# Sunscreen-tech/spf

Measured on AMD Instinct MI355X. Metric: programmable bootstraps/sec (CMUX gates/sec) at default 128-bit params, higher is better.
Workload: dtype f64

## Files before the change

spf_amd/csrc/spf_device.hpp:

```cpp
#pragma once
#include <hip/hip_runtime.h>
#include <stdint.h>

namespace spf {

struct c64 {
    double re, im;
};

typedef double f64x2_t __attribute__((ext_vector_type(2)));
typedef const f64x2_t __attribute__((address_space(1)))* gc64_ptr;
typedef const uint64_t __attribute__((address_space(1)))* gu64_cptr;
typedef uint64_t __attribute__((address_space(1)))* gu64_ptr;
__device__ __forceinline__ gc64_ptr global_view(const c64* p) { return (gc64_ptr)(uintptr_t)p; }
__device__ __forceinline__ gu64_cptr global_view(const uint64_t* p) { return (gu64_cptr)(uintptr_t)p; }
__device__ __forceinline__ gu64_ptr global_view(uint64_t* p) { return (gu64_ptr)(uintptr_t)p; }
__device__ __forceinline__ c64 gload(gc64_ptr p) { f64x2_t v = *p; return {v.x, v.y}; }
__device__ __forceinline__ c64 gload_stream(gc64_ptr p) { f64x2_t v = __builtin_nontemporal_load(p); return {v.x, v.y}; }

__device__ __forceinline__ c64 cadd(c64 a, c64 b) { return {a.re + b.re, a.im + b.im}; }
__device__ __forceinline__ c64 csub(c64 a, c64 b) { return {a.re - b.re, a.im - b.im}; }

__device__ __forceinline__ c64 cmul_nf(c64 a, c64 b)
{
    c64 o;
    o.re = a.re * b.re - a.im * b.im;
    o.im = a.re * b.im + a.im * b.re;
    return o;
}
__device__ __forceinline__ c64 cmul_nf_conj(c64 a, c64 b)
{
    c64 o;
    o.re = a.re * b.re + a.im * b.im;
    o.im = a.im * b.re - a.re * b.im;
    return o;
}

template <int DIR> __device__ __forceinline__ c64 cmul_tw(c64 a, c64 w)
{
    c64 o;
    if (DIR > 0) {
        double t1 = a.im * w.im;
        o.re = __builtin_fma(a.re, w.re, -t1);
        double t2 = a.im * w.re;
        o.im = __builtin_fma(a.re, w.im, t2);
    } else {
        double t1 = a.im * w.im;
        o.re = __builtin_fma(a.re, w.re, t1);
        double t2 = a.im * w.re;
        o.im = __builtin_fma(-a.re, w.im, t2);
    }
    return o;
}

constexpr double kSqrtHalf = 0.70710678118654752440;

template <int DIR> __device__ __forceinline__ void radix8(c64 (&v)[8])
{
    c64 s0 = cadd(v[0], v[4]), s1 = cadd(v[1], v[5]), s2 = cadd(v[2], v[6]), s3 = cadd(v[3], v[7]);
    c64 t0 = csub(v[0], v[4]), t1 = csub(v[1], v[5]), t2 = csub(v[2], v[6]), t3 = csub(v[3], v[7]);
    c64 t1w, t3w;
    if (DIR > 0) {
        double p1 = t1.re + t1.im, m1 = t1.im - t1.re;
        t1w.re = p1 * kSqrtHalf; t1w.im = m1 * kSqrtHalf;
        double p3 = t3.re + t3.im, m3 = t3.im - t3.re;
        t3w.re = m3 * kSqrtHalf; t3w.im = -(p3 * kSqrtHalf);
    } else {
        double p1 = t1.re + t1.im, m1 = t1.re - t1.im;
        t1w.re = m1 * kSqrtHalf; t1w.im = p1 * kSqrtHalf;
        double p3 = t3.re + t3.im, m3 = t3.re - t3.im;
        t3w.re = -(p3 * kSqrtHalf); t3w.im = m3 * kSqrtHalf;
    }
    c64 a0 = cadd(s0, s2), a1 = cadd(s1, s3), a2 = csub(s0, s2), d = csub(s1, s3);
    v[0] = cadd(a0, a1);
    v[4] = csub(a0, a1);
    c64 b0, b2;
    if (DIR > 0) {
        v[2] = {a2.re + d.im, a2.im - d.re};
        v[6] = {a2.re - d.im, a2.im + d.re};
        b0 = {t0.re + t2.im, t0.im - t2.re};
        b2 = {t0.re - t2.im, t0.im + t2.re};
    } else {
        v[2] = {a2.re - d.im, a2.im + d.re};
        v[6] = {a2.re + d.im, a2.im - d.re};
        b0 = {t0.re - t2.im, t0.im + t2.re};
        b2 = {t0.re + t2.im, t0.im - t2.re};
    }
    c64 b1 = cadd(t1w, t3w), e = csub(t1w, t3w);
    v[1] = cadd(b0, b1);
    v[5] = csub(b0, b1);
    if (DIR > 0) {
        v[3] = {b2.re + e.im, b2.im - e.re};
        v[7] = {b2.re - e.im, b2.im + e.re};
    } else {
        v[3] = {b2.re - e.im, b2.im + e.re};
        v[7] = {b2.re + e.im, b2.im - e.re};
    }
}

constexpr int kT1Off = 0;
constexpr int kT2Off = kT1Off + 7 * 64;
constexpr int kWCOff = kT2Off + 7 * 8;
constexpr int kTWOff = kWCOff + 512;
constexpr int kTableEntries = kTWOff + 1024;
constexpr int kTableBytes = kTableEntries * 16;
constexpr int kWaveBufBytes = 16384;

__device__ __forceinline__ void wave_lds_fence()
{
    asm volatile("s_waitcnt lgkmcnt(0)" ::: "memory");
}
__device__ __forceinline__ void compiler_fence() { asm volatile("" ::: "memory"); }
__device__ __forceinline__ void sched_fence()
{
    asm volatile("" ::: "memory");
    __builtin_amdgcn_sched_barrier(0);
}

template <int DIR, int PRE = 0>
__device__ __forceinline__ void fft512_single(c64 (&V)[8], char* buf, const c64* tab, int lane)
{
    const int hi3 = lane >> 3, lo3 = lane & 7;
    const int rd = 16 * (8 * lo3 + (hi3 ^ lo3));
    {
        c64 tw[PRE > 0 ? PRE : 1];
#pragma unroll
        for (int k = 0; k < PRE; k++) tw[k] = tab[kT1Off + k * 64 + lane];
        if constexpr (PRE > 0) compiler_fence();
        radix8<DIR>(V);
#pragma unroll
        for (int k1 = 1; k1 < 8; k1++)
            V[k1] = cmul_tw<DIR>(V[k1], (k1 - 1 < PRE) ? tw[k1 - 1 < PRE ? k1 - 1 : 0] : tab[kT1Off + (k1 - 1) * 64 + lane]);
    }
#pragma unroll
    for (int k1 = 0; k1 < 8; k1++)
        *reinterpret_cast<c64*>(buf + 16 * (64 * hi3 + 8 * k1 + (lo3 ^ k1))) = V[k1];
    wave_lds_fence();
    {
        c64 tw[PRE > 0 ? PRE : 1];
#pragma unroll
        for (int k = 0; k < PRE; k++) tw[k] = tab[kT2Off + k * 8 + hi3];
#pragma unroll
        for (int a = 0; a < 8; a++) V[a] = *reinterpret_cast<const c64*>(buf + 1024 * a + rd);
        if constexpr (PRE > 0) compiler_fence();
        radix8<DIR>(V);
#pragma unroll
        for (int c = 1; c < 8; c++)
            V[c] = cmul_tw<DIR>(V[c], (c - 1 < PRE) ? tw[c - 1 < PRE ? c - 1 : 0] : tab[kT2Off + (c - 1) * 8 + hi3]);
    }
    compiler_fence();
#pragma unroll
    for (int c = 0; c < 8; c++)
        *reinterpret_cast<c64*>(buf + 16 * (64 * hi3 + 8 * lo3 + (c ^ lo3))) = V[c];
    wave_lds_fence();
#pragma unroll
    for (int b = 0; b < 8; b++) V[b] = *reinterpret_cast<const c64*>(buf + 1024 * b + rd);
    radix8<DIR>(V);
    compiler_fence();
}

__device__ __forceinline__ void swap_halves32(double& a, double& b)
{
    uint32_t al = (uint32_t)__double2loint(a), ah = (uint32_t)__double2hiint(a);
    uint32_t bl = (uint32_t)__double2loint(b), bh = (uint32_t)__double2hiint(b);
    auto r0 = __builtin_amdgcn_permlane32_swap(al, bl, false, false);
    auto r1 = __builtin_amdgcn_permlane32_swap(ah, bh, false, false);
    a = __hiloint2double((int)r1[0], (int)r0[0]);
    b = __hiloint2double((int)r1[1], (int)r0[1]);
}
__device__ __forceinline__ void swap_rows16(double& a, double& b)
{
    uint32_t al = (uint32_t)__double2loint(a), ah = (uint32_t)__double2hiint(a);
    uint32_t bl = (uint32_t)__double2loint(b), bh = (uint32_t)__double2hiint(b);
    auto r0 = __builtin_amdgcn_permlane16_swap(al, bl, false, false);
    auto r1 = __builtin_amdgcn_permlane16_swap(ah, bh, false, false);
    a = __hiloint2double((int)r1[0], (int)r0[0]);
    b = __hiloint2double((int)r1[1], (int)r0[1]);
}
__device__ __forceinline__ void swap_lane8(double& a, double& b)
{
    constexpr int kRowRor8 = 0x128;
    int al = __double2loint(a), ah = __double2hiint(a);
    int bl = __double2loint(b), bh = __double2hiint(b);
    int nal = __builtin_amdgcn_update_dpp(al, bl, kRowRor8, 0xF, 0xC, false);
    int nah = __builtin_amdgcn_update_dpp(ah, bh, kRowRor8, 0xF, 0xC, false);
    int nbl = __builtin_amdgcn_update_dpp(bl, al, kRowRor8, 0xF, 0x3, false);
    int nbh = __builtin_amdgcn_update_dpp(bh, ah, kRowRor8, 0xF, 0x3, false);
    a = __hiloint2double(nah, nal);
    b = __hiloint2double(nbh, nbl);
}
__device__ __forceinline__ void lane_transpose_hi3(c64 (&V)[8])
{
#pragma unroll
    for (int r = 0; r < 4; r++) {
        swap_halves32(V[r].re, V[r + 4].re);
        swap_halves32(V[r].im, V[r + 4].im);
    }
#pragma unroll
    for (int r = 0; r < 8; r++) {
        if (r & 2) continue;
        swap_rows16(V[r].re, V[r + 2].re);
        swap_rows16(V[r].im, V[r + 2].im);
    }
#pragma unroll
    for (int r = 0; r < 8; r += 2) {
        swap_lane8(V[r].re, V[r + 1].re);
        swap_lane8(V[r].im, V[r + 1].im);
    }
}

template <int DIR>
__device__ __forceinline__ void fft512_pair_pipelined(c64 (&E)[8], c64 (&O)[8], char* bufE, char* bufO,
                                                      const c64* tab, int lane)
{
    const int hi3 = lane >> 3, lo3 = lane & 7;
    const int rd = 16 * (8 * lo3 + (hi3 ^ lo3));
    c64 tw1[7], tw2[7];
#pragma unroll
    for (int k1 = 1; k1 < 8; k1++) tw1[k1 - 1] = tab[kT1Off + (k1 - 1) * 64 + lane];
#pragma unroll
    for (int c = 1; c < 8; c++) tw2[c - 1] = tab[kT2Off + (c - 1) * 8 + hi3];
    compiler_fence();
    radix8<DIR>(E);
#pragma unroll
    for (int k1 = 1; k1 < 8; k1++) E[k1] = cmul_tw<DIR>(E[k1], tw1[k1 - 1]);
#pragma unroll
    for (int k1 = 0; k1 < 8; k1++)
        *reinterpret_cast<c64*>(bufE + 16 * (64 * hi3 + 8 * k1 + (lo3 ^ k1))) = E[k1];
    compiler_fence();
#pragma unroll
    for (int a = 0; a < 8; a++) E[a] = *reinterpret_cast<const c64*>(bufE + 1024 * a + rd);
    compiler_fence();
    radix8<DIR>(O);
#pragma unroll
    for (int k1 = 1; k1 < 8; k1++) O[k1] = cmul_tw<DIR>(O[k1], tw1[k1 - 1]);
#pragma unroll
    for (int k1 = 0; k1 < 8; k1++)
        *reinterpret_cast<c64*>(bufO + 16 * (64 * hi3 + 8 * k1 + (lo3 ^ k1))) = O[k1];
    compiler_fence();
#pragma unroll
    for (int a = 0; a < 8; a++) O[a] = *reinterpret_cast<const c64*>(bufO + 1024 * a + rd);
    compiler_fence();
    radix8<DIR>(E);
#pragma unroll
    for (int c = 1; c < 8; c++) E[c] = cmul_tw<DIR>(E[c], tw2[c - 1]);
#pragma unroll
    for (int c = 0; c < 8; c++)
        *reinterpret_cast<c64*>(bufE + 16 * (64 * hi3 + 8 * lo3 + (c ^ lo3))) = E[c];
    compiler_fence();
#pragma unroll
    for (int b = 0; b < 8; b++) E[b] = *reinterpret_cast<const c64*>(bufE + 1024 * b + rd);
    compiler_fence();
    radix8<DIR>(O);
#pragma unroll
    for (int c = 1; c < 8; c++) O[c] = cmul_tw<DIR>(O[c], tw2[c - 1]);
#pragma unroll
    for (int c = 0; c < 8; c++)
        *reinterpret_cast<c64*>(bufO + 16 * (64 * hi3 + 8 * lo3 + (c ^ lo3))) = O[c];
    compiler_fence();
#pragma unroll
    for (int b = 0; b < 8; b++) O[b] = *reinterpret_cast<const c64*>(bufO + 1024 * b + rd);
    compiler_fence();
    radix8<DIR>(E);
    radix8<DIR>(O);
    compiler_fence();
// ... 266 lines not shown
#pragma unroll
    for (int k = 0; k < 7; k++) tw[k] = tab[kT1Off + k * 64 + lane];
    compiler_fence();
    radix8<DIR>(A);
#pragma unroll
    for (int k1 = 1; k1 < 8; k1++) A[k1] = cmul_tw<DIR>(A[k1], tw[k1 - 1]);
    sched_fence();
    radix8_twr_spread<DIR>(B, tw, [&](int k) { store(A, k); });
    load(A, rd1);
    sched_fence();
#pragma unroll
    for (int c = 0; c < 7; c++) tw[c] = tab[kT2Off + c * 8 + hi3];
    compiler_fence();
    radix8_twr_spread<DIR>(A, tw, [&](int k) { store(B, k); });
    mid();
    load(B, rd1);
    sched_fence();
    radix8_twr_spread<DIR>(B, tw, [&](int k) { store(A, k); });
    load(A, rd2);
    sched_fence();
    if constexpr (XP == 2) {
        lane_transpose_hi3(B);
        radix8<DIR>(A);
        radix8<DIR>(B);
    } else {
        pair_tail_through_image<DIR>(A, B, store, load, rd2);
    }
    sched_fence();
}
template <int DIR, int XP = 2, class MID = no_hook>
__device__ __forceinline__ void fft512_pair1ts2(c64 (&A)[8], c64 (&B)[8], char* buf, const c64* tab, int lane, MID mid = MID())
{
    static_assert(XP == 2 || XP == 0, "exchange 2 of B in registers (2) or through the image behind A's (0)");
    const int hi3 = lane >> 3, lo3 = lane & 7;
    const uint32_t rd1 = 16 * (8 * lo3 + (hi3 ^ lo3));
    const uint32_t rd2 = 16 * (8 * hi3 + (hi3 ^ lo3));
    const uint32_t wbase = 16 * (64 * hi3 + lo3);
    char* wr[8];
#pragma unroll
    for (int r = 0; r < 8; r++) wr[r] = buf + ((wbase ^ (16 * r)) + 128 * r);
    auto store = [&](c64 (&X)[8], int k) { *reinterpret_cast<c64*>(wr[k]) = X[k]; };
    auto load = [&](c64 (&X)[8], uint32_t rd) {
#pragma unroll
        for (int a = 0; a < 8; a++) X[a] = *reinterpret_cast<const c64*>(buf + 1024 * a + rd);
    };
    c64 tw[7];
#pragma unroll
    for (int k = 0; k < 7; k++) tw[k] = tab[kT1Off + k * 64 + lane];
    compiler_fence();
    radix8<DIR>(A);
#pragma unroll
    for (int k1 = 1; k1 < 8; k1++) A[k1] = cmul_tw<DIR>(A[k1], tw[k1 - 1]);
    sched_fence();
    radix8_twr_spread2<DIR>(B, tw, [&](int k) { store(A, k); }, [&]() { load(A, rd1); });
    c64 tw2[7];
#pragma unroll
    for (int c = 0; c < 7; c++) tw2[c] = tab[kT2Off + c * 8 + hi3];
    compiler_fence();
    radix8_twr_spread2<DIR>(A, tw2, [&](int k) { store(B, k); }, [&]() { load(B, rd1); });
    mid();
    radix8_twr_spread2<DIR>(B, tw2, [&](int k) { store(A, k); }, [&]() { load(A, rd2); });
    if constexpr (XP == 2) {
        lane_transpose_hi3(B);
        radix8<DIR>(A);
        radix8<DIR>(B);
    } else {
        pair_tail_through_image<DIR>(A, B, store, load, rd2);
    }
    sched_fence();
}

__device__ __forceinline__ uint64_t f64_round_to_torus(double x)
{
    const double q = 18446744073709551616.0;
    const double q_div_2 = 9223372036854775808.0;
    double v = __builtin_round(x);
    double m = __builtin_fma(-__builtin_trunc(v * (1.0 / q)), q, v);
    double adj = (m >= q_div_2) ? -q : ((m <= -q_div_2) ? q : 0.0);
    m += adj;
    bool sat = m >= q_div_2;
    long long r = (long long)(sat ? 0.0 : m);
    r = sat ? 0x7FFFFFFFFFFFFFFFll : r;
    return (uint64_t)r;
}

__device__ __forceinline__ uint64_t f64_bigint_to_torus_bits(double v, uint32_t& sh_or, uint32_t& quirk_min)
{
    const uint64_t b = (uint64_t)__double_as_longlong(v);
    const uint32_t hi = (uint32_t)(b >> 32), lo = (uint32_t)b;
    const uint32_t sh = ((hi >> 20) & 0x7FFu) - 1075u;
    sh_or |= sh;
    const uint64_t m = ((uint64_t)((hi & 0xFFFFFu) | 0x100000u) << 32) | lo;
    uint64_t r = m << (sh & 63u);
    const uint32_t s32 = (uint32_t)((int32_t)hi >> 31);
    const uint64_t s = ((uint64_t)s32 << 32) | s32;
    r = (r ^ s) - s;
    const uint32_t q = (uint32_t)r | ((uint32_t)(r >> 32) ^ 0x80000000u) | ~s32;
    quirk_min = q < quirk_min ? q : quirk_min;
    return r;
}

__device__ __forceinline__ void torus_bits16_mantissa(const double (&tv)[16], uint64_t (&t)[16])
{
    uint32_t sh_or = 0, qmin = 0xFFFFFFFFu;
#pragma unroll
    for (int e = 0; e < 16; e++) t[e] = f64_bigint_to_torus_bits(tv[e], sh_or, qmin);
    if (!__all(sh_or < 64u && qmin != 0u)) {
#pragma unroll
        for (int e = 0; e < 16; e++) t[e] = f64_round_to_torus(tv[e]);
    }
}
__device__ __forceinline__ void torus_bits16(const double (&tv)[16], uint64_t (&t)[16])
{
    uint32_t emin = 0xFFFFFFFFu, emax = 0u;
    uint64_t quirk = 0;
#pragma unroll
    for (int e = 0; e < 16; e++) {
        const uint64_t b = (uint64_t)__double_as_longlong(tv[e]);
        const uint32_t hi = (uint32_t)(b >> 32);
        const uint32_t e11 = (hi >> 20) & 0x7FFu;
        emin = e11 < emin ? e11 : emin;
        emax = e11 > emax ? e11 : emax;
        const uint64_t r = b << ((e11 + 13u) & 63u);
        quirk |= __ballot((uint32_t)(r >> 32) == 0x80000000u);
        const uint32_t s32 = (uint32_t)((int32_t)hi >> 31);
        const uint64_t sg = ((uint64_t)s32 << 32) | s32;
        t[e] = (r ^ sg) - sg;
    }
    if (!__all(emin >= 1087u && emax <= 1138u) || quirk != 0) {
#pragma unroll
        for (int e = 0; e < 16; e++) t[e] = f64_round_to_torus(tv[e]);
    }
}
template <bool MANTISSA_FORM = false>
__device__ __forceinline__ void untwist_to_torus_bits(const c64 (&V)[8], const c64* twist_lds, uint64_t (&t)[16])
{
    double tv[16];
#pragma unroll
    for (int n1 = 0; n1 < 8; n1++) {
        c64 xs = {V[n1].re * (1.0 / 1024.0), V[n1].im * (1.0 / 1024.0)};
        c64 u = cmul_nf_conj(xs, twist_lds[64 * n1]);
        tv[n1] = u.re;
        tv[8 + n1] = u.im;
    }
    if constexpr (MANTISSA_FORM) torus_bits16_mantissa(tv, t);
    else torus_bits16(tv, t);
}
__device__ __forceinline__ uint64_t add_u32_to_u64(uint64_t a, uint32_t b)
{
    uint64_t out, carry;
    asm("v_mad_u64_u32 %0, %1, %2, 1, %3" : "=&v"(out), "=s"(carry) : "v"(b), "v"(a));
    return out;
}

template <bool TWIST_AT_ONCE = false>
__device__ __forceinline__ void untwist_sub_from_negated(const c64 (&V)[8], const c64* twist_lds, uint64_t (&nacc)[16])
{
    double tvn[16];
    c64 twf[TWIST_AT_ONCE ? 8 : 1];
    if constexpr (TWIST_AT_ONCE) {
#pragma unroll
        for (int n1 = 0; n1 < 8; n1++) twf[n1] = twist_lds[64 * n1];
        compiler_fence();
    }
#pragma unroll
    for (int n1 = 0; n1 < 8; n1++) {
        const c64 xs = V[n1];
        const c64 tw = TWIST_AT_ONCE ? twf[TWIST_AT_ONCE ? n1 : 0] : twist_lds[64 * n1];
        tvn[n1] = -(xs.re * tw.re) - xs.im * tw.im;
        tvn[8 + n1] = xs.re * tw.im - xs.im * tw.re;
    }
    uint32_t kmin = 0xFFFFFFFFu, kmax = 0u;
    int32_t qmin = 0x7FFFFFFF;
    uint64_t t[16];
#pragma unroll
    for (int e = 0; e < 16; e++) {
        const uint64_t b = (uint64_t)__double_as_longlong(tvn[e]);
        const uint32_t hi = (uint32_t)(b >> 32);
        const uint32_t k = hi << 1;
        kmin = k < kmin ? k : kmin;
        kmax = k > kmax ? k : kmax;
        const uint64_t r = b << (((hi >> 20) + 13u) & 63u);
        const int32_t rh = (int32_t)(uint32_t)(r >> 32);
        qmin = rh < qmin ? rh : qmin;
        const uint64_t sg = (uint64_t)((int64_t)b >> 63);
        t[e] = (r + sg) ^ sg;
    }
    if (__all(kmin >= (1087u << 21) && kmax < (1139u << 21) && qmin != (int32_t)0x80000000)) {
#pragma unroll
        for (int e = 0; e < 16; e++) nacc[e] += t[e];
    } else {
#pragma unroll
        for (int e = 0; e < 16; e++) nacc[e] -= f64_round_to_torus(-tvn[e]);
    }
}
__device__ __forceinline__ void untwist_to_torus_bits(const c64 (&V)[8], const c64 (&twist)[8], uint64_t (&t)[16])
{
    double tv[16];
#pragma unroll
    for (int n1 = 0; n1 < 8; n1++) {
        c64 xs = {V[n1].re * (1.0 / 1024.0), V[n1].im * (1.0 / 1024.0)};
        c64 u = cmul_nf_conj(xs, twist[n1]);
        tv[n1] = u.re;
        tv[8 + n1] = u.im;
    }
    torus_bits16(tv, t);
}


template <int L, int LOGB>
__device__ __forceinline__ uint32_t gadget_digits_packed(uint64_t x)
{
    static_assert(L * LOGB <= 32, "packed digits need L*LOGB <= 32");
    constexpr int shift = 64 - L * LOGB;
    uint32_t s = (uint32_t)(x >> shift) + (uint32_t)((x >> (shift - 1)) & 1);
    uint32_t packed = 0;
#pragma unroll
    for (int j = 0; j < L; j++) {
        uint32_t d = s & ((1u << LOGB) - 1);
        s >>= LOGB;
        s += d >> (LOGB - 1);
        packed |= d << (j * LOGB);
    }
    return packed;
}

__device__ __forceinline__ c64 twisted_digit_top32(uint32_t s_re, uint32_t s_im, int j, c64 tw)
{
    const int dre = j == 0 ? (int)(int16_t)(s_re & 0xFFFFu) : (int)(s_re + 0x8000u) >> 16;
    const int dim = j == 0 ? (int)(int16_t)(s_im & 0xFFFFu) : (int)(s_im + 0x8000u) >> 16;
    return cmul_nf({(double)dre, (double)dim}, tw);
}

template <int LOGB>
__device__ __forceinline__ c64 twisted_digit(uint32_t packed_re, uint32_t packed_im, int j, c64 tw)
{
    const int sh = j * LOGB;
    int dre = ((int)(packed_re << (32 - LOGB - sh))) >> (32 - LOGB);
    int dim = ((int)(packed_im << (32 - LOGB - sh))) >> (32 - LOGB);
    return cmul_nf({(double)dre, (double)dim}, tw);
}

}
```

spf_amd/csrc/spf_kernels.hpp:

```cpp
#pragma once
#include <type_traits>
#include "spf_device.hpp"

namespace spf {

constexpr int kN = 2048;
constexpr int kHalf = 1024;
constexpr int kWavesPerBlock = 4;

struct BlindRotateArgs {
    const uint64_t* lwe_in;
    const uint64_t* lut;
    size_t lut_stride;
    const c64* bsk;
    const c64* tables;
    uint64_t* out;
    size_t out_stride;
    uint32_t n;
    uint32_t B;
    uint32_t log_chi, log_v;
    uint64_t body_rotate;
    uint32_t sample_extract;
    uint64_t* stamps;
};

__device__ __forceinline__ uint32_t mod_switch_2n(uint64_t x, uint32_t log_chi, uint32_t log_v)
{
    const uint32_t log_modulus = 12;
    x = x << log_chi;
    uint32_t shift = 64 - (log_modulus - log_v);
    uint64_t round = (x >> (shift - 1)) & 1;
    x = x >> shift;
    return (uint32_t)(((x + round) & ((1u << log_modulus) - 1)) << log_v);
}

constexpr int kBskSlotBytes = 2 * kHalf * 16;

__device__ __forceinline__ void lds_dma_piece(const void* sbase, uint32_t voff, uint32_t lds)
{
    uint32_t saved_m0;
    asm volatile("s_mov_b32 %0, m0\n\ts_mov_b32 m0, %3\n\ts_nop 0\n\tglobal_load_lds_dwordx4 %1, %2\n\ts_mov_b32 m0, %0"
                 : "=&s"(saved_m0) : "v"(voff), "s"(sbase), "s"(lds) : "memory");
}
__device__ __forceinline__ uint32_t lds_address(const void* p)
{
    return (uint32_t)(size_t)(const __attribute__((address_space(3))) void*)p;
}

template <int NT>
__device__ __forceinline__ void table_image_dma(const c64* tables, char* smem, int tid, int wv)
{
    const char* src = reinterpret_cast<const char*>(tables);
    const uint32_t voff = (uint32_t)tid * 16u;
    const uint32_t dst = lds_address(smem) + (uint32_t)wv * 1024u;
    constexpr int kRow = NT * 16, kFull = kTableBytes / kRow, kRest = kTableBytes - kFull * kRow;
#pragma unroll
    for (int k = 0; k < kFull; k++) lds_dma_piece(src + k * kRow, voff, dst + k * kRow);
    if constexpr (kRest > 0) {
        if (tid * 16 < kRest) lds_dma_piece(src + kFull * kRow, voff, dst + kFull * kRow);
    }
}

__device__ __forceinline__ void pair_barrier_w()
{
    asm volatile("s_waitcnt lgkmcnt(0)" ::: "memory");
    __builtin_amdgcn_s_barrier();
    asm volatile("" ::: "memory");
}

constexpr int kBlindRotate2pLds = kTableBytes + 4 * kWaveBufBytes + 2 * kBskSlotBytes;

template <int PRIO>
__device__ __forceinline__ void young_prio(uint32_t flag) {
    uint32_t tmp;
    if constexpr (PRIO != 0)
        asm volatile("v_readfirstlane_b32 %0, %1\n\ts_cmp_eq_u32 %0, 0\n\ts_cbranch_scc1 .Lprio%=\n\ts_setprio 1\n.Lprio%=:" : "=&s"(tmp) : "v"(flag) : "scc");
    else
        asm volatile("v_readfirstlane_b32 %0, %1\n\ts_cmp_eq_u32 %0, 0\n\ts_cbranch_scc1 .Lprio%=\n\ts_setprio 0\n.Lprio%=:" : "=&s"(tmp) : "v"(flag) : "scc");
}

#ifndef SPF_PRIO_SCHED_EVEN
#define SPF_PRIO_SCHED_EVEN "----00----10--1-----"
#endif
#ifndef SPF_PRIO_SCHED_MIX
#define SPF_PRIO_SCHED_MIX "----1-----1---10-00-"
#endif
template <int MIX> constexpr char prio_sched_at(int i) { return MIX ? SPF_PRIO_SCHED_MIX[i] : SPF_PRIO_SCHED_EVEN[i]; }
static_assert(sizeof(SPF_PRIO_SCHED_EVEN) == 21 && sizeof(SPF_PRIO_SCHED_MIX) == 21, "20 schedule points");

#ifndef SPF_PAIR_E0
#define SPF_PAIR_E0 fft512_pair1ts2
#endif
#ifndef SPF_PAIR_E1
#define SPF_PAIR_E1 fft512_pair1ts
#endif
#ifndef SPF_PAIR_EI
#define SPF_PAIR_EI fft512_pair1ts2
#endif
#ifndef SPF_PAIR_M0
#define SPF_PAIR_M0 fft512_pair1ts
#endif
#ifndef SPF_PAIR_M1
#define SPF_PAIR_M1 fft512_pair1ts
#endif
#ifndef SPF_PAIR_MI
#define SPF_PAIR_MI fft512_pair1ts
#endif
#ifndef SPF_BR_OPT
#define SPF_BR_OPT 6
#endif
#ifndef SPF_BR_OPT_MIX
#define SPF_BR_OPT_MIX 10
#endif
#ifndef SPF_BR2_OPT
#define SPF_BR2_OPT 6
#endif
template <int L, int LOGB, int OPT, int W, int CTS = 4, int MIX = 1>
__device__ __forceinline__ void blind_rotate2p_body(const BlindRotateArgs& a, char* smem)
{
    constexpr int XP = (OPT & 1) ? 1 : ((OPT & 2) ? 2 : 0);
#ifdef SPF_STAMPS
    uint64_t st_acc[12] = {0, 0, 0, 0, 0, 0, 0, 0, 0, 0, 0, 0};
    uint64_t st_prev = __builtin_amdgcn_s_memtime();
#define STAMP(i) do { uint64_t t_ = __builtin_amdgcn_s_memtime(); st_acc[i] += t_ - st_prev; st_prev = t_; } while (0)
#else
#define STAMP(i) do { } while (0)
#endif
    static_assert(L == 2 && LOGB == 16, "two 16-bit digits, taken straight from the rounded top word and processed as a pair");
    constexpr int NT = 128 * CTS;
    c64* tab = reinterpret_cast<c64*>(smem);
    const int tid = threadIdx.x;
    const int lane = tid & 63;
    const int wv = __builtin_amdgcn_readfirstlane(tid >> 6);
    const int cslot = wv >> 1;
    constexpr int w = W;
    char* tile = smem + kTableBytes + cslot * kWaveBufBytes;
    char* mine = tile + w * 8192;
    char* theirs = tile + (w ^ 1) * 8192;
    char* bskring = smem + kTableBytes + CTS * kWaveBufBytes;

    {
        const double2* src = reinterpret_cast<const double2*>(a.tables);
        double2* dst = reinterpret_cast<double2*>(smem);
        for (int i = tid; i < kTableEntries; i += NT) dst[i] = src[i];
    }

    const uint32_t ct_raw = blockIdx.x * CTS + cslot;
    const bool owns_output = ct_raw < a.B;
    const uint32_t ct = owns_output ? ct_raw : a.B - 1;
    const uint64_t* lwe = a.lwe_in + (size_t)ct * (a.n + 1);
    const uint64_t* lut = a.lut + (size_t)ct * a.lut_stride;

    const uint32_t total_chunks = 2 * a.n;
    const uint32_t dma_voff = (uint32_t)tid * 16u;
    const uint32_t dma_dst = lds_address(bskring) + wv * 1024;
    constexpr int kPieces = 2 * kBskSlotBytes / 1024, NW = 2 * CTS;
    static_assert(kPieces % NW == 0, "every wave copies the same number of 1 KiB pieces of a chunk (a three-per-workgroup shape would not)");
    auto ring_dma = [&](uint32_t chunk) {
        const char* src = reinterpret_cast<const char*>(a.bsk) +
                          (size_t)__builtin_amdgcn_readfirstlane(chunk) * (2 * kBskSlotBytes);
#pragma unroll
        for (int k = 0; k < 2 * kBskSlotBytes / (NT * 16); k++)
            lds_dma_piece(src + k * NT * 16, dma_voff, dma_dst + k * NT * 16);
    };
    ring_dma(0);

    auto coef2 = [&](int e) -> int { return (e >> 3) * 1024 + (e & 7) * 128 + 2 * lane + w; };

    uint64_t acc[2][16];
    {
        uint32_t bt = mod_switch_2n(lwe[a.n] + a.body_rotate, a.log_chi, a.log_v);
#pragma unroll
        for (int p = 0; p < 2; p++)
#pragma unroll
            for (int e = 0; e < 16; e++) {
                uint32_t idx = (uint32_t)coef2(e) + bt;
                uint64_t v = lut[p * kN + (idx & (kN - 1))];
                acc[p][e] = ((idx >> 11) & 1) ? v : (uint64_t)0 - v;
            }
    }
    __syncthreads();
    constexpr bool PRIO = CTS == 4;
    const uint32_t is_young = __builtin_amdgcn_readfirstlane(wv >= CTS ? 1u : 0u);
    uint32_t opaque_zero;
    asm volatile("s_mov_b32 %0, 0" : "=s"(opaque_zero));
    auto rendezvous = [&]() {
        do {
            pair_barrier_w();
        } while (opaque_zero != 0);
    };
#define SPF_PRIO_POINT(i) do { if constexpr (PRIO) { if constexpr (prio_sched_at<MIX>(i) == '1') young_prio<1>(is_young); \
                                                      else if constexpr (prio_sched_at<MIX>(i) == '0') young_prio<0>(is_young); } } while (0)
    auto rendezvous_if_mixing = [&]() {
        do {
            if constexpr (MIX) pair_barrier_w();
            else asm volatile("" ::: "memory");
        } while (opaque_zero != 0);
    };

    uint64_t* stage_mine = reinterpret_cast<uint64_t*>(mine);
    const c64* twist = tab + kTWOff + w * 512 + lane;
    const c64* wc = tab + kWCOff + 256 * w + lane;
    uint64_t a_next = lwe[0];
    uint32_t chunk = 0;
    auto stage = [&](int p) {
#pragma unroll
        for (int e = 0; e < 16; e++) stage_mine[(e >> 3) * 512 + (e & 7) * 64 + lane] = acc[p][e];
    };
    for (uint32_t step = 0; step < a.n; step++) {
        const uint32_t at = mod_switch_2n(a_next, a.log_chi, a.log_v);
        a_next = lwe[step + 1];
        STAMP(11);

        c64 prod[2][8];

#pragma unroll
        for (int p = 0; p < 2; p++, chunk++) {
            if (p == 0) SPF_PRIO_POINT(0); else SPF_PRIO_POINT(8);
            stage(p);
            if (p == 0) SPF_PRIO_POINT(1);
            rendezvous_if_mixing();
            STAMP(0);
            if (p == 0) SPF_PRIO_POINT(2); else SPF_PRIO_POINT(9);
            uint32_t dig[16];
            {
                const uint32_t t0 = (uint32_t)(2 * lane + w) + 2 * kN - at;
                const char* region = tile + (t0 & 1) * 8192;
                uint32_t T0 = (t0 + 2048u) << 20;
                asm volatile("" : "+v"(T0));
                uint64_t gin[16];
#pragma unroll
                for (int e = 0; e < 16; e++) {
                    const uint32_t t = t0 + (e >> 3) * 1024 + (e & 7) * 128;
                    gin[e] = *reinterpret_cast<const uint64_t*>(region + ((t << 2) & 0x1FF8u));
                }
                sched_fence();
#pragma unroll
                for (int e = 0; e < 16; e++) {
                    const uint32_t m32 = (uint32_t)((int32_t)(T0 + (uint32_t)(((e >> 3) * 1024 + (e & 7) * 128) << 20)) >> 31);
                    const uint64_t m = ((uint64_t)m32 << 32) | m32;
                    uint32_t k32 = 0x80000000u - m32;
                    dig[e] = (uint32_t)(((gin[e] ^ m) + add_u32_to_u64(acc[p][e], k32)) >> 32);
                }
            }
            c64 VV[2][8];
            constexpr bool kTwistBatch = MIX || CTS != 4;
            if constexpr (kTwistBatch) {
                c64 twf[8];
#pragma unroll
                for (int n1 = 0; n1 < 8; n1++) twf[n1] = twist[64 * n1];
                compiler_fence();
#pragma unroll
                for (int n1 = 0; n1 < 8; n1++) {
                    VV[0][n1] = twisted_digit_top32(dig[n1], dig[8 + n1], 0, twf[n1]);
                    VV[1][n1] = twisted_digit_top32(dig[n1], dig[8 + n1], 1, twf[n1]);
                }
            } else {
#pragma unroll
                for (int n1 = 0; n1 < 8; n1++) {
                    const c64 tw = twist[64 * n1];
                    VV[0][n1] = twisted_digit_top32(dig[n1], dig[8 + n1], 0, tw);
                    VV[1][n1] = twisted_digit_top32(dig[n1], dig[8 + n1], 1, tw);
                }
            }
            STAMP(1);
            if (p == 0) SPF_PRIO_POINT(3);
            rendezvous_if_mixing();
            STAMP(2);
            if (p == 0) SPF_PRIO_POINT(4); else SPF_PRIO_POINT(10);
            if (p == 1) ring_dma(chunk);
            if constexpr (MIX) {
                if (p == 0) SPF_PAIR_M0<+1, XP>(VV[0], VV[1], mine, tab, lane, [&]() { SPF_PRIO_POINT(17); });
                else SPF_PAIR_M1<+1, XP>(VV[0], VV[1], mine, tab, lane, [&]() { SPF_PRIO_POINT(18); });
            } else {
                if (p == 0) SPF_PAIR_E0<+1, XP>(VV[0], VV[1], mine, tab, lane, [&]() { SPF_PRIO_POINT(17); });
                else SPF_PAIR_E1<+1, XP>(VV[0], VV[1], mine, tab, lane, [&]() { SPF_PRIO_POINT(18); });
            }
            STAMP(3);
            if (p == 0) SPF_PRIO_POINT(5);
            if constexpr (w == 0) {
#pragma unroll
                for (int j = 0; j < 2; j++)
#pragma unroll
                    for (int i = 0; i < 4; i++) reinterpret_cast<c64*>(mine)[(j * 4 + i) * 64 + lane] = VV[j][4 + i];
            } else {
#pragma unroll
                for (int j = 0; j < 2; j++)
#pragma unroll
                    for (int i = 0; i < 4; i++) reinterpret_cast<c64*>(mine)[(j * 4 + i) * 64 + lane] = VV[j][i];
            }
            if (p == 1) SPF_PRIO_POINT(11);
#ifdef SPF_STAMPS
            STAMP(4);
            asm volatile("s_waitcnt vmcnt(0)" ::: "memory");
            STAMP(2);
#endif
            asm volatile("s_waitcnt vmcnt(0)" ::: "memory");
            __syncthreads();
            STAMP(4);
            if (p == 0) SPF_PRIO_POINT(6); else SPF_PRIO_POINT(12);
            if constexpr (w == 0) {
#pragma unroll
                for (int j = 0; j < 2; j++)
#pragma unroll
                    for (int i = 0; i < 4; i++) {
                        const c64 in = reinterpret_cast<const c64*>(theirs)[(j * 4 + i) * 64 + lane];
                        const c64 t = cmul_tw<+1>(in, wc[64 * i]);
                        const c64 Ei = VV[j][i];
                        VV[j][i] = cadd(Ei, t);
                        VV[j][i + 4] = csub(Ei, t);
                    }
            } else {
#pragma unroll
                for (int j = 0; j < 2; j++)
#pragma unroll
                    for (int i = 0; i < 4; i++) {
                        const c64 Ei = reinterpret_cast<const c64*>(theirs)[(j * 4 + i) * 64 + lane];
                        const c64 t = cmul_tw<+1>(VV[j][4 + i], wc[64 * i]);
                        VV[j][i] = cadd(Ei, t);
                        VV[j][i + 4] = csub(Ei, t);
                    }
            }
            STAMP(5);
#pragma unroll
            for (int j = 0; j < 2; j++) {
                const c64* row = reinterpret_cast<const c64*>(bskring + (1 - j) * kBskSlotBytes) + 256 * w + lane;
                constexpr int KD = (OPT & 4) ? 2 : 3;
                c64 kb[KD][2];
                auto key2 = [&](int grp, c64 (&dst)[2]) {
#pragma unroll
                    for (int i = 0; i < 2; i++) {
                        const int r = (grp * 2 + i) & 7, q = grp >> 2;
                        dst[i] = row[q * kHalf + 64 * (r & 3) + 512 * (r >> 2)];
                    }
                };
                key2(0, kb[0]);
                if constexpr (KD >= 3) key2(1, kb[1]);
#pragma unroll
                for (int grp = 0; grp < 8; grp++) {
                    if (grp + KD - 1 < 8) key2(grp + KD - 1, kb[(grp + KD - 1) % KD]);
                    compiler_fence();
#pragma unroll
                    for (int i = 0; i < 2; i++) {
                        const int r = (grp * 2 + i) & 7, q = grp >> 2;
                        const c64 k = kb[grp % KD][i];
                        const bool first = p == 0 && j == 0;
                        double re = __builtin_fma(k.re, VV[j][r].re, first ? 0.0 : prod[q][r].re);
                        double im = __builtin_fma(k.re, VV[j][r].im, first ? 0.0 : prod[q][r].im);
                        prod[q][r].re = __builtin_fma(-k.im, VV[j][r].im, re);
                        prod[q][r].im = __builtin_fma(k.im, VV[j][r].re, im);
                    }
                }
            }
            STAMP(6);
            if (p == 0) SPF_PRIO_POINT(7);
            __syncthreads();
            STAMP(7);
            if (p == 1) SPF_PRIO_POINT(13);
        }

        c64 WW[2][8];
#pragma unroll
        for (int q = 0; q < 2; q++)
#pragma unroll
            for (int i = 0; i < 4; i++) {
                const c64 wci = wc[64 * i];
                WW[q][i] = cadd(prod[q][i], prod[q][i + 4]);
                WW[q][4 + i] = cmul_tw<-1>(csub(prod[q][i], prod[q][i + 4]), wci);
            }
        if constexpr ((OPT & 8) != 0) {
            c64* slot_mine = reinterpret_cast<c64*>(bskring + wv * 8192);
            const c64* slot_theirs = reinterpret_cast<const c64*>(bskring + (wv ^ 1) * 8192);
            if constexpr (w == 0) {
#pragma unroll
                for (int q = 0; q < 2; q++)
#pragma unroll
                    for (int i = 0; i < 4; i++) slot_mine[(q * 4 + i) * 64 + lane] = WW[q][4 + i];
            } else {
#pragma unroll
                for (int q = 0; q < 2; q++)
#pragma unroll
                    for (int i = 0; i < 4; i++) slot_mine[(q * 4 + i) * 64 + lane] = WW[q][i];
            }
            rendezvous();
            if constexpr (w == 0) {
#pragma unroll
                for (int q = 0; q < 2; q++)
#pragma unroll
                    for (int i = 0; i < 4; i++) WW[q][4 + i] = slot_theirs[(q * 4 + i) * 64 + lane];
            } else {
#pragma unroll
                for (int q = 0; q < 2; q++)
#pragma unroll
                    for (int i = 0; i < 4; i++) WW[q][i] = slot_theirs[(q * 4 + i) * 64 + lane];
            }
            asm volatile("s_waitcnt lgkmcnt(0)" ::: "memory");
            STAMP(8);
            SPF_PRIO_POINT(14);
            if (chunk < total_chunks) {
                const char* src = reinterpret_cast<const char*>(a.bsk) +
                                  (size_t)__builtin_amdgcn_readfirstlane(chunk) * (2 * kBskSlotBytes);
                const uint32_t lane16 = (uint32_t)lane * 16u;
                const uint32_t ring0 = lds_address(bskring);
#pragma unroll
                for (int k = 0; k < 8; k++)
                    lds_dma_piece(src + (wv ^ 1) * 8192 + k * 1024, lane16, ring0 + (wv ^ 1) * 8192 + k * 1024);
                constexpr int kRest = (2 * kBskSlotBytes - 2 * CTS * 8192) / 1024;
                static_assert(kRest % NW == 0, "every wave copies the same number of 1 KiB pieces of the rest of the ring");
#pragma unroll
                for (int k = 0; k < kRest / NW; k++)
                    lds_dma_piece(src + 2 * CTS * 8192 + (wv * (kRest / NW) + k) * 1024, lane16,
                                  ring0 + 2 * CTS * 8192 + (wv * (kRest / NW) + k) * 1024);
            }
        } else {
            if constexpr (w == 0) {
    #pragma unroll
                for (int q = 0; q < 2; q++)
    #pragma unroll
                    for (int i = 0; i < 4; i++) reinterpret_cast<c64*>(mine)[(q * 4 + i) * 64 + lane] = WW[q][4 + i];
            } else {
    #pragma unroll
                for (int q = 0; q < 2; q++)
    #pragma unroll
                    for (int i = 0; i < 4; i++) reinterpret_cast<c64*>(mine)[(q * 4 + i) * 64 + lane] = WW[q][i];
            }
            rendezvous();
            if constexpr (w == 0) {
    #pragma unroll
                for (int q = 0; q < 2; q++)
    #pragma unroll
                    for (int i = 0; i < 4; i++) WW[q][4 + i] = reinterpret_cast<const c64*>(theirs)[(q * 4 + i) * 64 + lane];
            } else {
    #pragma unroll
                for (int q = 0; q < 2; q++)
    #pragma unroll
                    for (int i = 0; i < 4; i++) WW[q][i] = reinterpret_cast<const c64*>(theirs)[(q * 4 + i) * 64 + lane];
            }
            rendezvous();
            STAMP(8);
            SPF_PRIO_POINT(14);
            if (chunk < total_chunks) ring_dma(chunk);
        }
        if constexpr (MIX) SPF_PAIR_MI<-1, XP>(WW[0], WW[1], mine, tab, lane, [&]() { SPF_PRIO_POINT(19); });
        else SPF_PAIR_EI<-1, XP>(WW[0], WW[1], mine, tab, lane, [&]() { SPF_PRIO_POINT(19); });
        STAMP(9);
        SPF_PRIO_POINT(15);
#pragma unroll
        for (int q = 0; q < 2; q++) {
            untwist_sub_from_negated<CTS != 4>(WW[q], twist, acc[q]);
            if (q == 0) SPF_PRIO_POINT(16);
        }
        STAMP(10);
    }
#ifdef SPF_STAMPS
    if (a.stamps && lane == 0) {
#pragma unroll
        for (int i = 0; i < 12; i++) a.stamps[((size_t)blockIdx.x * (2 * CTS) + wv) * 16 + i] = st_acc[i];
    }
#endif
#undef STAMP
#undef SPF_PRIO_POINT

    if (!owns_output) return;
    uint64_t* out = a.out + (size_t)ct * a.out_stride;
#pragma unroll
    for (int p = 0; p < 2; p++)
#pragma unroll
        for (int e = 0; e < 16; e++) acc[p][e] = (uint64_t)0 - acc[p][e];
    if (!a.sample_extract) {
#pragma unroll
        for (int p = 0; p < 2; p++)
#pragma unroll
            for (int e = 0; e < 16; e++) out[p * kN + coef2(e)] = acc[p][e];
    } else {
#pragma unroll
        for (int e = 0; e < 16; e++) {
            int c = coef2(e);
            if (c == 0) {
                out[0] = acc[0][e];
                out[kN] = acc[1][e];
            } else {
                out[kN - c] = (uint64_t)0 - acc[0][e];
            }
        }
    }
}


template <int L, int LOGB, int OPT, int MIX = 1>
__global__ __launch_bounds__(512, 2) void blind_rotate2p_kernel(BlindRotateArgs a)
{
    extern __shared__ __attribute__((aligned(16))) char smem[];
    if (__builtin_amdgcn_readfirstlane(threadIdx.x >> 6) & 1) blind_rotate2p_body<L, LOGB, OPT, 1, 4, MIX>(a, smem);
    else blind_rotate2p_body<L, LOGB, OPT, 0, 4, MIX>(a, smem);
}

constexpr int kBlindRotate2p2Lds = kTableBytes + 2 * kWaveBufBytes + 2 * kBskSlotBytes;
template <int L, int LOGB, int OPT, int MIX = 1>
__global__ __launch_bounds__(256, 1) void blind_rotate2p2_kernel(BlindRotateArgs a)
{
    extern __shared__ __attribute__((aligned(16))) char smem[];
    if (__builtin_amdgcn_readfirstlane(threadIdx.x >> 6) & 1) blind_rotate2p_body<L, LOGB, OPT, 1, 2, MIX>(a, smem);
    else blind_rotate2p_body<L, LOGB, OPT, 0, 2, MIX>(a, smem);
}

__global__ void scale_bootstrap_key_kernel(const double* key, double* scaled, size_t n, unsigned int* bad)
{
    bool flagged = false;
    for (size_t i = (size_t)blockIdx.x * blockDim.x + threadIdx.x; i < n; i += (size_t)gridDim.x * blockDim.x) {
        const double v = key[i];
        const double m = __builtin_fabs(v);
        if (!(m == 0.0 || (m >= 0x1p-900 && m < 0x1p1000))) flagged = true;
        scaled[i] = v * 0x1p-10;
    }
    if (flagged) atomicOr(bad, 1u);
}

constexpr int kBlindRotate8Lds = kTableBytes + 8 * 8192 + 4 * 16384;

template <int L, int LOGB, int W, int J, int MIX>
__device__ __forceinline__ void blind_rotate8_body(const BlindRotateArgs& a, char* smem)
{
    static_assert(L == 2 && L * LOGB <= 32, "two digits, one per wave of a pair");
    c64* tab = reinterpret_cast<c64*>(smem);
    const int tid = threadIdx.x;
    const int lane = tid & 63;
    const int wv = __builtin_amdgcn_readfirstlane(tid >> 6);
    constexpr int w = W, j = J;
    const int h = (wv >> 1) & 1;
    auto image = [&](int ww, int hh, int jj) -> char* { return smem + kTableBytes + ((jj * 2 + hh) * 2 + ww) * 8192; };
    char* mine = image(w, h, j);
    char* partner = image(w ^ 1, h, j);
    auto spectra = [&](int ww, int hh) -> char* { return smem + kTableBytes + 8 * 8192 + (hh * 2 + ww) * 16384; };
    auto wg_barrier = [&]() {
        asm volatile("s_waitcnt lgkmcnt(0)" ::: "memory");
        __builtin_amdgcn_s_barrier();
        asm volatile("" ::: "memory");
    };
    {
        const double2* src = reinterpret_cast<const double2*>(a.tables);
        double2* dst = reinterpret_cast<double2*>(smem);
        for (int i = tid; i < kTableEntries; i += 512) dst[i] = src[i];
    }
    const uint32_t ct = blockIdx.x;
    const uint64_t* lwe = a.lwe_in + (size_t)ct * (a.n + 1);
    const uint64_t* lut = a.lut + (size_t)ct * a.lut_stride;
    auto coef2 = [&](int e) -> int { return (e >> 3) * 1024 + (e & 7) * 128 + 2 * lane + w; };

    uint64_t acc[16];
    if constexpr (J == 0) {
        uint32_t bt = mod_switch_2n(lwe[a.n] + a.body_rotate, a.log_chi, a.log_v);
#pragma unroll
        for (int e = 0; e < 16; e++) {
            uint32_t idx = (uint32_t)coef2(e) + bt;
            uint64_t v = lut[h * kN + (idx & (kN - 1))];
            acc[e] = ((idx >> 11) & 1) ? v : (uint64_t)0 - v;
        }
    }
    __syncthreads();

    const c64* twist_lds = tab + kTWOff + w * 512 + lane;
    const c64* wc_lds = tab + kWCOff + 256 * w + lane;

    c64 key[2][2][4];
    const c64* key_base = a.bsk + h * kHalf + 256 * w + lane + 128 * j;
    const c64* key_next = key_base;
    auto request_keys = [&](auto piece_c) {
        constexpr int piece = decltype(piece_c)::value;
        constexpr int p = piece >> 1, jj = piece & 1;
        const c64* row = key_next + (size_t)(p * L + (L - 1 - jj)) * (2 * kHalf);
#pragma unroll
        for (int q = 0; q < 4; q++) key[p][jj][q] = row[64 * (q & 1) + 512 * (q >> 1)];
    };
#define SPF_KEY_PIECE(i) request_keys(std::integral_constant<int, i>{})
    SPF_KEY_PIECE(0); SPF_KEY_PIECE(1); SPF_KEY_PIECE(2); SPF_KEY_PIECE(3);
    uint64_t a_next = lwe[0];
#ifdef SPF_STAMPS
    uint64_t st_acc[12] = {0, 0, 0, 0, 0, 0, 0, 0, 0, 0, 0, 0};
    uint64_t st_prev = __builtin_amdgcn_s_memtime();
#define STAMP8(i) do { uint64_t t_ = __builtin_amdgcn_s_memtime(); st_acc[i] += t_ - st_prev; st_prev = t_; } while (0)
#else
#define STAMP8(i) do { } while (0)
#endif
    auto cmux_step = [&](uint32_t step, auto last_c) {
        constexpr bool LAST = decltype(last_c)::value;
        const uint32_t at = mod_switch_2n(a_next, a.log_chi, a.log_v);
        a_next = lwe[step + 1];
        c64 V[8];
        uint4* digits1 = reinterpret_cast<uint4*>(image(w, h, 1));
        if constexpr (J == 0) {
            uint64_t* stage = reinterpret_cast<uint64_t*>(spectra(w, h));
#pragma unroll
            for (int e = 0; e < 16; e++) stage[(e >> 3) * 512 + (e & 7) * 64 + lane] = acc[e];
            STAMP8(0);
            if constexpr (MIX) wg_barrier();
            else compiler_fence();
            STAMP8(1);
            const uint32_t t0 = (uint32_t)(2 * lane + w) + 2 * kN - at;
            const char* src = spectra((int)(t0 & 1), h);
            uint32_t T0 = (t0 + 2048u) << 20;
            asm volatile("" : "+v"(T0));
            uint64_t gin[16];
#pragma unroll
            for (int e = 0; e < 16; e++) {
                const uint32_t t = t0 + (e >> 3) * 1024 + (e & 7) * 128;
                gin[e] = *reinterpret_cast<const uint64_t*>(src + ((t << 2) & 0x1FF8u));
            }
            c64 twist[8];
#pragma unroll
            for (int n1 = 0; n1 < 8; n1++) twist[n1] = twist_lds[64 * n1];
            sched_fence();
            uint32_t dig[16];
#pragma unroll
            for (int e = 0; e < 16; e++) {
                const uint32_t m32 = (uint32_t)((int32_t)(T0 + (uint32_t)(((e >> 3) * 1024 + (e & 7) * 128) << 20)) >> 31);
                const uint64_t m = ((uint64_t)m32 << 32) | m32;
                const uint32_t k32 = 0x80000000u - m32;
                const uint32_t s = (uint32_t)(((gin[e] ^ m) + add_u32_to_u64(acc[e], k32)) >> 32);
                dig[e] = (s & 0xFFFFu) | ((s + 0x8000u) & 0xFFFF0000u);
            }
            static_assert(LOGB == 16, "digit 1 of the real and of the imaginary element share a 32-bit word");
            uint32_t pk[8];
#pragma unroll
            for (int n1 = 0; n1 < 8; n1++) pk[n1] = (dig[n1] >> 16) | (dig[8 + n1] & 0xFFFF0000u);
            digits1[lane] = uint4{pk[0], pk[1], pk[2], pk[3]};
            digits1[64 + lane] = uint4{pk[4], pk[5], pk[6], pk[7]};
            wg_barrier();
#pragma unroll
            for (int n1 = 0; n1 < 8; n1++) V[n1] = twisted_digit<LOGB>(dig[n1], dig[8 + n1], 0, twist[n1]);
        } else {
            STAMP8(0);
            if constexpr (MIX) wg_barrier();
            c64 twist[8];
#pragma unroll
            for (int n1 = 0; n1 < 8; n1++) twist[n1] = twist_lds[64 * n1];
// ... 953 lines not shown
```

Before: 106,800.

## Pack accumulator coefficient pairs into 128-bit vectors for staging and gadget reads

Stores each lane's accumulator as eight 2-wide u64 vectors that pair coefficient e with e+1024, so the LDS staging writes and the rotated-tile reads become 128-bit accesses instead of 64-bit ones. When reading, the two halves are swapped with cndmask based on the rotation sign bit, which changes the staging layout and the address computation together. The goal is fewer LDS instructions per step. In exchange it adds inline-asm select work and may raise register pressure or cause LDS bank conflicts.

```diff
diff --git a/spf_amd/csrc/spf_device.hpp b/spf_amd/csrc/spf_device.hpp
--- a/spf_amd/csrc/spf_device.hpp
+++ b/spf_amd/csrc/spf_device.hpp
@@ -111,6 +111,7 @@
     asm volatile("s_waitcnt lgkmcnt(0)" ::: "memory");
 }
 __device__ __forceinline__ void compiler_fence() { asm volatile("" ::: "memory"); }
+typedef uint64_t u64x2 __attribute__((ext_vector_type(2)));
 __device__ __forceinline__ void sched_fence()
 {
     asm volatile("" ::: "memory");
@@ -683,11 +684,21 @@
     asm("v_mad_u64_u32 %0, %1, %2, 1, %3" : "=&v"(out), "=s"(carry) : "v"(b), "v"(a));
     return out;
 }
-
-template <bool TWIST_AT_ONCE = false>
-__device__ __forceinline__ void untwist_sub_from_negated(const c64 (&V)[8], const c64* twist_lds, uint64_t (&nacc)[16])
-{
-    double tvn[16];
+__device__ __forceinline__ void select_pair_halves(u64x2 pair, uint32_t sel, uint64_t& first, uint64_t& second)
+{
+    typedef uint32_t u32x4 __attribute__((ext_vector_type(4)));
+    const u32x4 q = __builtin_bit_cast(u32x4, pair);
+    uint32_t f0, f1, s0, s1;
+    asm("v_cmp_gt_i32_e32 vcc, 0, %4\n\tv_cndmask_b32_e32 %0, %5, %7, vcc\n\tv_cndmask_b32_e32 %1, %6, %8, vcc\n\t"
+        "v_cndmask_b32_e32 %2, %7, %5, vcc\n\tv_cndmask_b32_e32 %3, %8, %6, vcc"
+        : "=&v"(f0), "=&v"(f1), "=&v"(s0), "=&v"(s1) : "v"(sel), "v"(q[0]), "v"(q[1]), "v"(q[2]), "v"(q[3]) : "vcc");
+    first = ((uint64_t)f1 << 32) | f0;
+    second = ((uint64_t)s1 << 32) | s0;
+}
+
+template <bool TWIST_AT_ONCE>
+__device__ __forceinline__ bool negated_untwist_terms(const c64 (&V)[8], const c64* twist_lds, double (&tvn)[16], uint64_t (&t)[16])
+{
     c64 twf[TWIST_AT_ONCE ? 8 : 1];
     if constexpr (TWIST_AT_ONCE) {
 #pragma unroll
@@ -703,7 +714,6 @@
     }
     uint32_t kmin = 0xFFFFFFFFu, kmax = 0u;
     int32_t qmin = 0x7FFFFFFF;
-    uint64_t t[16];
 #pragma unroll
     for (int e = 0; e < 16; e++) {
         const uint64_t b = (uint64_t)__double_as_longlong(tvn[e]);
@@ -717,12 +727,32 @@
         const uint64_t sg = (uint64_t)((int64_t)b >> 63);
         t[e] = (r + sg) ^ sg;
     }
-    if (__all(kmin >= (1087u << 21) && kmax < (1139u << 21) && qmin != (int32_t)0x80000000)) {
+    return __all(kmin >= (1087u << 21) && kmax < (1139u << 21) && qmin != (int32_t)0x80000000);
+}
+template <bool TWIST_AT_ONCE = false>
+__device__ __forceinline__ void untwist_sub_from_negated(const c64 (&V)[8], const c64* twist_lds, uint64_t (&nacc)[16])
+{
+    double tvn[16];
+    uint64_t t[16];
+    if (negated_untwist_terms<TWIST_AT_ONCE>(V, twist_lds, tvn, t)) {
 #pragma unroll
         for (int e = 0; e < 16; e++) nacc[e] += t[e];
     } else {
 #pragma unroll
         for (int e = 0; e < 16; e++) nacc[e] -= f64_round_to_torus(-tvn[e]);
+    }
+}
+template <bool TWIST_AT_ONCE = false>
+__device__ __forceinline__ void untwist_sub_from_negated(const c64 (&V)[8], const c64* twist_lds, u64x2 (&nacc)[8])
+{
+    double tvn[16];
+    uint64_t t[16];
+    if (negated_untwist_terms<TWIST_AT_ONCE>(V, twist_lds, tvn, t)) {
+#pragma unroll
+        for (int n1 = 0; n1 < 8; n1++) nacc[n1] += u64x2{t[n1], t[8 + n1]};
+    } else {
+#pragma unroll
+        for (int n1 = 0; n1 < 8; n1++) nacc[n1] -= u64x2{f64_round_to_torus(-tvn[n1]), f64_round_to_torus(-tvn[8 + n1])};
     }
 }
 __device__ __forceinline__ void untwist_to_torus_bits(const c64 (&V)[8], const c64 (&twist)[8], uint64_t (&t)[16])
diff --git a/spf_amd/csrc/spf_kernels.hpp b/spf_amd/csrc/spf_kernels.hpp
--- a/spf_amd/csrc/spf_kernels.hpp
+++ b/spf_amd/csrc/spf_kernels.hpp
@@ -167,7 +167,7 @@
 
     auto coef2 = [&](int e) -> int { return (e >> 3) * 1024 + (e & 7) * 128 + 2 * lane + w; };
 
-    uint64_t acc[2][16];
+    u64x2 acc[2][8];
     {
         uint32_t bt = mod_switch_2n(lwe[a.n] + a.body_rotate, a.log_chi, a.log_v);
 #pragma unroll
@@ -176,7 +176,7 @@
             for (int e = 0; e < 16; e++) {
                 uint32_t idx = (uint32_t)coef2(e) + bt;
                 uint64_t v = lut[p * kN + (idx & (kN - 1))];
-                acc[p][e] = ((idx >> 11) & 1) ? v : (uint64_t)0 - v;
+                acc[p][e & 7][e >> 3] = ((idx >> 11) & 1) ? v : (uint64_t)0 - v;
             }
     }
     __syncthreads();
@@ -198,14 +198,14 @@
         } while (opaque_zero != 0);
     };
 
-    uint64_t* stage_mine = reinterpret_cast<uint64_t*>(mine);
+    u64x2* stage_mine = reinterpret_cast<u64x2*>(mine);
     const c64* twist = tab + kTWOff + w * 512 + lane;
     const c64* wc = tab + kWCOff + 256 * w + lane;
     uint64_t a_next = lwe[0];
     uint32_t chunk = 0;
     auto stage = [&](int p) {
 #pragma unroll
-        for (int e = 0; e < 16; e++) stage_mine[(e >> 3) * 512 + (e & 7) * 64 + lane] = acc[p][e];
+        for (int m = 0; m < 8; m++) stage_mine[m * 64 + lane] = acc[p][m];
     };
     for (uint32_t step = 0; step < a.n; step++) {
         const uint32_t at = mod_switch_2n(a_next, a.log_chi, a.log_v);
@@ -228,19 +228,24 @@
                 const char* region = tile + (t0 & 1) * 8192;
                 uint32_t T0 = (t0 + 2048u) << 20;
                 asm volatile("" : "+v"(T0));
-                uint64_t gin[16];
-#pragma unroll
-                for (int e = 0; e < 16; e++) {
-                    const uint32_t t = t0 + (e >> 3) * 1024 + (e & 7) * 128;
-                    gin[e] = *reinterpret_cast<const uint64_t*>(region + ((t << 2) & 0x1FF8u));
+                u64x2 gpair[8];
+#pragma unroll
+                for (int m = 0; m < 8; m++) {
+                    const uint32_t t = t0 + m * 128;
+                    gpair[m] = *reinterpret_cast<const u64x2*>(region + ((t << 3) & 0x1FF0u));
                 }
                 sched_fence();
+                uint64_t gin[16];
+#pragma unroll
+                for (int m = 0; m < 8; m++) {
+                    select_pair_halves(gpair[m], (T0 + (uint32_t)((m * 128) << 20)) << 1, gin[m], gin[8 + m]);
+                }
 #pragma unroll
                 for (int e = 0; e < 16; e++) {
                     const uint32_t m32 = (uint32_t)((int32_t)(T0 + (uint32_t)(((e >> 3) * 1024 + (e & 7) * 128) << 20)) >> 31);
                     const uint64_t m = ((uint64_t)m32 << 32) | m32;
                     uint32_t k32 = 0x80000000u - m32;
-                    dig[e] = (uint32_t)(((gin[e] ^ m) + add_u32_to_u64(acc[p][e], k32)) >> 32);
+                    dig[e] = (uint32_t)(((gin[e] ^ m) + add_u32_to_u64(acc[p][e & 7][e >> 3], k32)) >> 32);
                 }
             }
             c64 VV[2][8];
@@ -466,21 +471,21 @@
 #pragma unroll
     for (int p = 0; p < 2; p++)
 #pragma unroll
-        for (int e = 0; e < 16; e++) acc[p][e] = (uint64_t)0 - acc[p][e];
+        for (int m = 0; m < 8; m++) acc[p][m] = (u64x2)(0) - acc[p][m];
     if (!a.sample_extract) {
 #pragma unroll
         for (int p = 0; p < 2; p++)
 #pragma unroll
-            for (int e = 0; e < 16; e++) out[p * kN + coef2(e)] = acc[p][e];
+            for (int e = 0; e < 16; e++) out[p * kN + coef2(e)] = acc[p][e & 7][e >> 3];
     } else {
 #pragma unroll
         for (int e = 0; e < 16; e++) {
             int c = coef2(e);
             if (c == 0) {
-                out[0] = acc[0][e];
-                out[kN] = acc[1][e];
+                out[0] = acc[0][e & 7][e >> 3];
+                out[kN] = acc[1][e & 7][e >> 3];
             } else {
-                out[kN - c] = (uint64_t)0 - acc[0][e];
+                out[kN - c] = (uint64_t)0 - acc[0][e & 7][e >> 3];
             }
         }
     }
```

Result: slower. 103,600 (-3.1%).
